# vt-asaplab/vPIN

Measured on AMD Instinct MI355X. Metric: R1CS constraints/sec, whole Spartan SNARK (sat proof + SPARK evaluation proof; vPIN point-mult + point-add instances), higher is better.
Workload: dtype u256 (integers mod q and mod p = 2^255-19, 32-bit limbs); 1 GPU; vPIN LeNet trace (layers L1..L7): 12 SNARKs per step; inputs=resident in HBM, parallelism=one trace per rank x 1 rank(s), no collective; 4 stream(s) per rank, table_slot_bytes=128

## Files before the change

### include/vpin_hip.h

```cpp
#ifndef VPIN_HIP_H
#define VPIN_HIP_H
#include <stddef.h>
#include <stdint.h>

#ifdef __cplusplus
extern "C" {
#endif

#define VPIN_OK 0
#define VPIN_EINVAL (-1)
#define VPIN_ENODEV (-2)
#define VPIN_ENOMEM (-3)
#define VPIN_EHIP (-4)
#define VPIN_ESHAPE (-5)
#define VPIN_EVERIFY (-6)

typedef struct vpin_ctx vpin_ctx;
typedef struct vpin_table vpin_table;

const char* vpin_strerror(int code);
const char* vpin_last_error(void);
int vpin_crash_line_set(const char* line, size_t n);
int vpin_abi_version(void);

// ... 39 lines not shown
int vpin_sc_quad_bind_round(vpin_ctx* ctx, vpin_table* A, vpin_table* B, const uint8_t r[32],
                            uint8_t out_e0_e2[64]);

int vpin_eq_table(vpin_ctx* ctx, const uint8_t* r, int ell, vpin_table** out);

int vpin_eq_suffix_tables(vpin_ctx* ctx, const uint8_t* tau, int ell, vpin_table** out);
int vpin_sc_cubic3_round(vpin_ctx* ctx, const vpin_table* pyramid, int ell, int level, vpin_table* Az,
                         vpin_table* Bz, vpin_table* Cz, uint8_t out_S0_S2_S3[96]);
int vpin_sc_cubic3_bind_round(vpin_ctx* ctx, const vpin_table* pyramid, int ell, int level, vpin_table* Az,
                              vpin_table* Bz, vpin_table* Cz, const uint8_t r[32], uint8_t out_S0_S2_S3[96]);
int vpin_sc_cubic3_lead_round(vpin_ctx* ctx, const vpin_table* pyramid, int ell, int level, vpin_table* Az,
                              vpin_table* Bz, vpin_table* Cz, const uint8_t* r, uint8_t out[96]);
int vpin_spark_batched_round(vpin_ctx* ctx, vpin_table* forest, size_t n, int ncirc, int level, size_t len,
                             const vpin_table* E, size_t e_off, const uint8_t* r, int lead, const vpin_table* derefs,
                             const vpin_table* vals, vpin_table* scratch, int first_fold, uint8_t* out);

typedef struct vpin_gens vpin_gens;
int vpin_gens_create(vpin_ctx* ctx, const uint8_t* gens_xyzt, size_t nb, vpin_gens** out);
int vpin_gens_map_stream(vpin_ctx* ctx, const uint8_t* stream64, size_t nb, uint8_t* out_xyzt);
int vpin_gens_shared(vpin_ctx* ctx, const char* label, const uint8_t* gens_xyzt, size_t nb, size_t budget_gb,
                     const vpin_gens** out);
void vpin_gens_shared_clear(void);
size_t vpin_gens_shared_bytes(int device);
void vpin_gens_free(vpin_ctx* ctx, vpin_gens* g);
size_t vpin_gens_count(const vpin_gens* g);
int vpin_gens_layout(const vpin_gens* g, size_t out[6]);
size_t vpin_gens_entry_bytes(void);
int vpin_hyrax_commit(vpin_ctx* ctx, const vpin_gens* g, const vpin_table* Z, const uint8_t* blinds,
                      size_t L, size_t blind_base, uint8_t* out_compressed );
int vpin_hyrax_commit_rows(vpin_ctx* ctx, const vpin_gens* g, const vpin_table* Z, size_t L, size_t row0, size_t nrows,
// ... 200 lines not shown
```

### vpin_amd/csrc/sc_dev.h

```cpp
#pragma once
#include <cstring>

#include "ctx.h"

namespace vpin {

#ifndef VPIN_SC_MIN_WAVES
#define VPIN_SC_MIN_WAVES 3
#endif
constexpr int kBlock = 256;
constexpr int kMinWaves = VPIN_SC_MIN_WAVES;
constexpr int kMaxBlocksCap = 16384;
inline int max_blocks() {
  static const int n = [] { const char* e = getenv("VPIN_SC_BLOCKS"); int v = e ? atoi(e) : 1024; return v < 1 ? 1 : v > kMaxBlocksCap ? kMaxBlocksCap : v; }();
  return n;
}


__device__ __forceinline__ fq comb_cubic(const fq& a, const fq& b, const fq& c, const fq& d) {
  return fq_mul(a, fq_sub(fq_mul(b, c), d));
}

template <int K>
struct Acc;
// ... 65 lines not shown
    fqw_mac(w[1], E, Y);
#ifndef VPIN_LAZY_NO_FLUSH
    if (++n == 7) flush(e);
#endif
#endif
  }
  __device__ __forceinline__ void flush(fq* e) {
    if (n == 0) return;
    e[0] = fq_add(e[0], fqw_reduce(w[0]));
    e[1] = fq_add(e[1], fqw_reduce(w[1]));
    fqw_zero(w[0]); fqw_zero(w[1]);
    n = 0;
  }
};

template <>
struct Acc<2> {
  static constexpr int NE = 2;
  fq e[2];
  __device__ __forceinline__ void init() { e[0] = e[1] = fq_zero(); }
  __device__ __forceinline__ void add_pair(fq* p, const fq* d) {
    e[0] = fq_add(e[0], fq_mul(p[0], p[1]));
#pragma unroll
    for (int k = 0; k < 2; k++) p[k] = fq_add(fq_add(p[k], d[k]), d[k]);
    e[1] = fq_add(e[1], fq_mul(p[0], p[1]));
  }
};

template <int K>
struct Tabs {
// ... 89 lines not shown
```

### vpin_amd/csrc/spark.cpp

```cpp
#include <cstdio>

#include "host/prover_common.h"
#include "gadget_dev.h"
#include "spark_dev.h"

namespace {

using namespace vpin_host;
using namespace vpin_prover;

static bool spark_trace() { static const bool on = getenv("VPIN_SPARK_TRACE") != nullptr; return on; }
struct TraceSpan {
  const char* name; Clock::time_point t0;
  explicit TraceSpan(const char* n) : name(n), t0(Clock::now()) {}
  ~TraceSpan() { if (spark_trace()) fprintf(stderr, "[spark] %-28s %8.3f ms\n", name, secs(t0, Clock::now()) * 1e3); }
};


struct SparkGens {
  std::vector<Point> g;
  std::map<size_t, std::unique_ptr<PcGens>> views;
};

static void spark_cache_free(vpin_ctx* c) {
// ... 216 lines not shown
  std::vector<Fq> dotp[3];
};

static void write_batched(Writer& w, const Batched& b) {
  w.u64(b.polys.size());
  for (size_t l = 0; l < b.polys.size(); l++) {
    w.u64(b.polys[l].size() / 3);
    for (size_t j = 0; j < b.polys[l].size() / 3; j++) w_scalars(w, &b.polys[l][3 * j], 3);
    w_scalars(w, b.claims_left[l].data(), b.claims_left[l].size());
    w_scalars(w, b.claims_right[l].data(), b.claims_right[l].size());
  }
  for (int k = 0; k < 3; k++) w_scalars(w, b.dotp[k].data(), b.dotp[k].size());
}

static inline size_t pyramid_offset(int ell, int k) { return ((size_t)1 << ell) - ((size_t)2 << (ell - k)); }

struct DotpCtx {
  const vpin_spark_decomm* d;
  const vpin::fq* comb_derefs;
  vpin::fq* scratch;
  Fq claims[6];
};

static int batched_prove(vpin_ctx* c, vpin::SparkForest& f, DotpCtx* dotp, Transcript& tr, Batched& out, std::vector<Fq>& rand,
                         const DistPlan* pl = nullptr, int npc_all = 0) {
  const int npc = pl ? npc_all : f.ncirc, ndotp = dotp ? 6 : 0;
  const bool is_mem = pl && npc_all == 4;
  const int nl = f.ncirc;
  const std::vector<int> no_halves;
  const std::vector<int>& my_halves = pl ? pl->dotp_of[pl->rank] : no_halves;
// ... 96 lines not shown
      for (auto& x : rho_inv) lead_ok = lead_ok && !x.is_zero();
      if (lead_ok) {
        std::vector<Fq> pre(k);
        Fq acc = one;
        for (int j = 0; j < k; j++) { pre[j] = acc; acc = acc * rho_inv[j]; }
        acc = acc.invert();
        for (int j = k - 1; j >= 0; j--) { Fq t = acc * rho_inv[j]; rho_inv[j] = acc * pre[j]; acc = t; }
      }
      Fq cn = Fq::zero();
      for (int t = 0; t < npc; t++) cn = cn + claims[t] * coeffs[t];
      const size_t tail_pairs = lead_ok ? vpin::spark_tail_pairs() : 0;
      if (pl && tail_pairs == 0) {
        vpin::set_last_error("one proof over several GPUs needs the persistent tail rounds", hipErrorUnknown);
        return VPIN_ESHAPE;
      }
      bool tail_on = false;
      int tail_j0 = 0;
      const int ninst = nl + ndl_here;
      if (fine) { auto t = Clock::now(); t_setup += secs(tl0, t); tl0 = t; }
      for (int j = 0; j < k; j++) {
        const size_t len = j == 0 ? h : (h >> (j - 1));
        const vpin::fq* E = runs ? pyr->d + pyramid_offset(k, j + 1) : nullptr;
        const uint8_t* rprev = j ? B(&r[j - 1]) : nullptr;
        if (!tail_on && (h >> (j + 1)) <= tail_pairs) {
          if (runs && (rc = vpin::spark_tail_launch(c, &f, layer_id, k, j, len, pyr->d, rprev, ndl_here ? dotp->d->N : 0,
                                                    ndl_here ? dotp->d->vals : nullptr,
                                                    ndl_here ? dotp->comb_derefs : nullptr, ndl_here ? dotp->scratch : nullptr,
                                                    halves, ndl_here)))
            return rc;
          tail_on = true;
          tail_j0 = j;
        }
        const Fq* res = nullptr;
        if (tail_on) {
          if (runs) {
            if ((rc = vpin::spark_tail_wait(c, j - tail_j0, ninst, nl))) return rc;
            res = reinterpret_cast<const Fq*>(vpin::spark_tail_sums(c));
          }
        } else if (runs) {
          if ((rc = vpin::spark_prod_round(c, &f, layer_id, len, E, rprev, ndl_here, lead_ok))) return rc;
          if (ndl_here && (rc = vpin::spark_dotp_round(c, dotp->d->N, dotp->d->vals, dotp->comb_derefs, dotp->scratch, len, j == 1, rprev, halves, ndl_here))) return rc;
          if ((rc = vpin::spark_wait_flag(c))) return rc;
          res = reinterpret_cast<const Fq*>(c->h_spark);
        }
        if (pl) {
          for (int t = 0; t < nl; t++) memcpy(&pack[3 * (size_t)t], res + 3 * (size_t)t, 96);
          for (int i = 0; i < ndl_here; i++) memcpy(&pack[3 * (size_t)(nl + i)], res + 3 * (size_t)((tail_on ? nl : 12) + i), 96);
          if ((rc = dist_exchange(c, *pl, is_mem, with_dotp, pack.data(), 3, res_all.data(),
                                  is_mem ? (tail_on ? "mem_tail_round" : "mem_round") : (tail_on ? "ops_tail_round" : "ops_round"))))
            return rc;
          res = res_all.data();
        }
        if (fine) { auto t = Clock::now(); (j == 0 ? t_first : t_rounds) += secs(tl0, t); if (k >= 11) fprintf(stderr, " w%.1f", secs(tl0, t) * 1e6); tl0 = t; }
        const Fq rho = rand[j], omr = one - rho;
        Fq S0 = Fq::zero(), S2 = Fq::zero(), S3 = Fq::zero(), T1 = Fq::zero(), Sinf = Fq::zero();
        if (lead_ok) {
          for (int t = 0; t < npc; t++) { S0 = S0 + res[3 * t] * coeffs[t]; Sinf = Sinf + res[3 * t + 1] * coeffs[t]; }
          T1 = (cn - omr * S0) * rho_inv[j];
// ... 810 lines not shown
  return 8 * 6 + 8 + 32 * ((size_t)1 << (s.v_ops / 2)) + 8 + 32 * ((size_t)1 << (s.v_mem / 2));
}

size_t vpin_snark_proof_max_bytes(const vpin_r1cs* inst) {
  if (!inst) return 0;
  Shape s = shape_of(inst->num_cons, inst->num_vars, inst->nnz);
  const size_t lgN = log2z(s.N), lgM = log2z(s.M);
  size_t b = vpin_sat_proof_max_bytes(inst->num_cons, inst->num_vars) + 96;
  b += 8 + 32 * ((size_t)1 << (s.v_derefs / 2)) + 64 * 32;
  b += lgN * (lgN * 104 + 64 + 24 * 32 + 64) + 18 * 32 + 64;
  b += lgM * (lgM * 104 + 64 + 8 * 32 + 64) + 64;
  b += 3 * (16 + 64 * 40 + 128 + 64) + 40 * 32 + 1024;
  return b;
}

int vpin_spark_prepare(vpin_ctx* c, size_t num_cons, size_t num_vars, size_t max_nnz) {
  if (!c || !vpin::is_pow2(num_cons) || !vpin::is_pow2(num_vars) || max_nnz == 0) return VPIN_EINVAL;
  (void)hipSetDevice(c->device);
  const size_t nnz[3] = {max_nnz, max_nnz, max_nnz};
  const Shape s = shape_of(num_cons, num_vars, nnz);
  const PcGens* g = nullptr;
  int rc = get_view(c, std::max(s.v_ops, s.v_mem), &g);
  if (!rc) {
    auto* sg = static_cast<SparkGens*>(c->spark_cache);
    std::vector<size_t> idx;
    for (size_t ell : {s.v_ops, s.v_mem, s.v_derefs}) {
      const size_t R = (size_t)1 << (ell - ell / 2);
      if (R + 1 < sg->g.size()) { idx.push_back(R); idx.push_back(R + 1); }
    }
#pragma omp parallel for schedule(dynamic, 1) num_threads(host_threads())
// ... 312 lines not shown
```

### vpin_amd/csrc/spark.hip

```cpp
#include <chrono>
#include <cstdlib>

#include "mailbox_dev.h"
#include "sc_dev.h"
#include "spark_dev.h"

namespace vpin {

__device__ __forceinline__ fq fq_r2() {
  fq r;
  r.v[0] = 0x449c0f01u; r.v[1] = 0xa40611e3u; r.v[2] = 0x68859347u; r.v[3] = 0xd00e1ba7u;
  r.v[4] = 0x17f5be65u; r.v[5] = 0xceec73d2u; r.v[6] = 0x7c309a3du; r.v[7] = 0x0399411bu;
  return r;
}
__device__ __forceinline__ fq fq_raw_u32(uint32_t x) {
  fq r = fq_zero();
  r.v[0] = x;
  return r;
}

__global__ __launch_bounds__(kBlock) void u32_to_fq_kernel(const uint32_t* __restrict__ src, fq* __restrict__ dst, size_t n) {
  const fq r2 = fq_r2();
  for (size_t i = (size_t)blockIdx.x * kBlock + threadIdx.x; i < n; i += (size_t)gridDim.x * kBlock) {
    uint32_t x = src[i];
// ... 7 lines not shown
  const int s = blockIdx.y;
  fq* dst = comb + (size_t)s * N;
  if (s >= 6) {
    for (size_t i = (size_t)blockIdx.x * kBlock + threadIdx.x; i < N; i += (size_t)gridDim.x * kBlock) fq_store(dst + i, fq_zero());
    return;
  }
  const uint32_t* a = idx + (size_t)(s < 3 ? s : 3 + s) * N;
  const fq* mem = s < 3 ? mem_rx : mem_ry;
  for (size_t i = (size_t)blockIdx.x * kBlock + threadIdx.x; i < N; i += (size_t)gridDim.x * kBlock)
    fq_store(dst + i, fq_load(mem + a[i]));
}

struct HashParams { fq r, r2, r2_boost, gamma; };
struct CircIds { int v[12]; };

__global__ __launch_bounds__(kBlock) void hash_ops_kernel(const uint32_t* __restrict__ idx, const fq* __restrict__ derefs, size_t N,
                                                          HashParams hp, fq* __restrict__ forest) {
  const int side = blockIdx.y / 3, m = blockIdx.y % 3;
  const uint32_t* addr = idx + (size_t)(side * 6 + m) * N;
  const uint32_t* ts = idx + (size_t)(side * 6 + 3 + m) * N;
  const fq* val = derefs + (size_t)(side * 3 + m) * N;
  fq* rd = forest + (size_t)(side * 6 + m) * 2 * N;
  fq* wr = forest + (size_t)(side * 6 + 3 + m) * 2 * N;
  const fq r2c = fq_r2();
  for (size_t i = (size_t)blockIdx.x * kBlock + threadIdx.x; i < N; i += (size_t)gridDim.x * kBlock) {
    fq h = fq_sub(fq_mul(fq_load(val + i), hp.r), hp.gamma);
    uint32_t a = addr[i], t = ts[i];
    if (a) h = fq_add(h, fq_mul(fq_raw_u32(a), r2c));
    if (t) h = fq_add(h, fq_mul(fq_raw_u32(t), hp.r2_boost));
    fq_store(rd + i, h);
    fq_store(wr + i, fq_add(h, hp.r2));
  }
}

__global__ __launch_bounds__(kBlock) void hash_mem_kernel(const uint32_t* __restrict__ audit_ts, const fq* __restrict__ mem_rx,
                                                          const fq* __restrict__ mem_ry, size_t M, HashParams hp,
                                                          fq* __restrict__ forest) {
  const int side = blockIdx.y;
  const fq* mem = side ? mem_ry : mem_rx;
  const uint32_t* ts = audit_ts + (size_t)side * M;
  fq* init = forest + (size_t)(2 * side) * 2 * M;
  fq* audit = forest + (size_t)(2 * side + 1) * 2 * M;
  const fq r2c = fq_r2();
  for (size_t i = (size_t)blockIdx.x * kBlock + threadIdx.x; i < M; i += (size_t)gridDim.x * kBlock) {
    fq h = fq_sub(fq_mul(fq_load(mem + i), hp.r), hp.gamma);
    if (i) h = fq_add(h, fq_mul(fq_raw_u32((uint32_t)i), r2c));
// ... 113 lines not shown
__global__ __launch_bounds__(kBlock) void take_strided_kernel(const fq* __restrict__ src, size_t nloc, size_t r0, size_t step,
                                                              fq* __restrict__ dst) {
  for (size_t k = (size_t)blockIdx.x * kBlock + threadIdx.x; k < nloc; k += (size_t)gridDim.x * kBlock)
    fq_store(dst + k, fq_load(src + r0 + k * step));
}

__global__ __launch_bounds__(kBlock) void tree_level_kernel(fq* __restrict__ forest, size_t stride, size_t src_off, size_t dst_off,
                                                            size_t h) {
  fq* t = forest + (size_t)blockIdx.y * stride;
  const fq* src = t + src_off;
  fq* dst = t + dst_off;
  for (size_t i = (size_t)blockIdx.x * kBlock + threadIdx.x; i < h; i += (size_t)gridDim.x * kBlock)
    fq_store(dst + i, fq_mul(fq_load(src + i), fq_load(src + h + i)));
}

__global__ __launch_bounds__(kBlock) void tree_level3_kernel(fq* __restrict__ forest, size_t stride, size_t src_off, size_t d1_off,
                                                             size_t d2_off, size_t d3_off, size_t h) {
  fq* t = forest + (size_t)blockIdx.y * stride;
  const fq* src = t + src_off;
  fq *d1 = t + d1_off, *d2 = t + d2_off, *d3 = t + d3_off;
  const size_t q = h / 4;
  for (size_t i = (size_t)blockIdx.x * kBlock + threadIdx.x; i < q; i += (size_t)gridDim.x * kBlock) {
    const fq a0 = fq_mul(fq_load(src + i), fq_load(src + h + i));
    const fq a1 = fq_mul(fq_load(src + q + i), fq_load(src + h + q + i));
    const fq a2 = fq_mul(fq_load(src + 2 * q + i), fq_load(src + h + 2 * q + i));
    const fq a3 = fq_mul(fq_load(src + 3 * q + i), fq_load(src + h + 3 * q + i));
    fq_store(d1 + i, a0); fq_store(d1 + q + i, a1); fq_store(d1 + 2 * q + i, a2); fq_store(d1 + 3 * q + i, a3);
    const fq b0 = fq_mul(a0, a2), b1 = fq_mul(a1, a3);
    fq_store(d2 + i, b0); fq_store(d2 + q + i, b1);
    fq_store(d3 + i, fq_mul(b0, b1));
  }
}

constexpr int kTopBlock = 1024;
__global__ __launch_bounds__(kTopBlock) void tree_top_kernel(fq* __restrict__ forest, size_t stride, size_t n2, size_t h0) {
  fq* t = forest + (size_t)blockIdx.x * stride;
  for (size_t h = h0; h >= 1; h >>= 1) {
    const fq* src = t + (n2 - 4 * h);
    fq* dst = t + (n2 - 2 * h);
    if (threadIdx.x < h) fq_store(dst + threadIdx.x, fq_mul(fq_load(src + threadIdx.x), fq_load(src + h + threadIdx.x)));
    __syncthreads();
  }
}


// ... 63 lines not shown
    }
  }
}


__device__ __forceinline__ void fold_pd2(const fq* src, fq* dst, size_t i, size_t q, const fq& r, fq& p, fq& d) {
  fq a0 = fq_load(src + i), a1 = fq_load(src + 2 * q + i);
  fq b0 = fq_load(src + q + i), b1 = fq_load(src + 3 * q + i);
  p = fq_add(a0, fq_mul(r, fq_sub(a1, a0)));
  fq hi = fq_add(b0, fq_mul(r, fq_sub(b1, b0)));
  fq_store(dst + i, p);
  fq_store(dst + q + i, hi);
  d = fq_sub(hi, p);
}

template <bool BIND, bool LEAD, bool BIG = false>
__global__ __launch_bounds__(kBlock, kMinWaves) void prod_round_kernel(fq* __restrict__ forest, size_t stride, size_t off, size_t h,
                                                                       const fq* __restrict__ E, size_t pairs, fq r, fq_const rc,
                                                                       Finisher fin) {
  __shared__ __attribute__((aligned(16))) uint32_t tt[8][8];
  if (BIND && LEAD) {
    if (threadIdx.x < 64) tt[threadIdx.x >> 3][threadIdx.x & 7] = rc.tt[threadIdx.x >> 3][threadIdx.x & 7];
    __syncthreads();
  }
  fq* A = forest + (size_t)blockIdx.y * stride + off;
  fq* B = A + h;
  Acc<4> acc;
  acc.init();
  LeadAcc lacc;
  if (LEAD) lacc.init();
  for (size_t i = (size_t)blockIdx.x * kBlock + threadIdx.x; i < pairs; i += (size_t)gridDim.x * kBlock) {
    fq u[3], p1, d1, p2, d2;
    if (BIND && LEAD) { fold_pd_c(A, i, pairs, tt, p1, d1); fold_pd_c(B, i, pairs, tt, p2, d2); }
    else if (BIND) { fold_pd(A, i, pairs, r, p1, d1); fold_pd(B, i, pairs, r, p2, d2); }
    else { load_pd(A, i, pairs, p1, d1); load_pd(B, i, pairs, p2, d2); }
    if (LEAD) {
      lacc.add(acc.e, fq_load(E + i), fq_mul(p1, p2), fq_mul(d1, d2));
    } else {
      acc.stage_bc(u, p1, d1, p2, d2);
      acc.stage_e(u, fq_load(E + i));
    }
  }
  if (LEAD) lacc.flush(acc.e);
  finish_block(acc.e, fin);
}

struct DotpPtrs { const fq* src[3]; fq* dst[3]; size_t src_stride[3]; };

template <bool BIND>
__global__ __launch_bounds__(kBlock, kMinWaves) void dotp_round_kernel(const fq* __restrict__ derefs, const fq* __restrict__ vals,
                                                                       size_t N, fq* __restrict__ scratch, bool from_scratch,
                                                                       size_t pairs, fq r, Finisher fin, CircIds kmap) {
  const int k = kmap.v[blockIdx.y], m = k >> 1, half = k & 1;
  const size_t hN = N / 2, q4 = N / 4;
  const fq* src[3];
  fq* dst[3];
#pragma unroll
  for (int t = 0; t < 3; t++) dst[t] = scratch + (size_t)(3 * blockIdx.y + t) * q4;
  if (from_scratch) {
// ... 291 lines not shown
  for (int m = 0; m < 3; m++) {
    const int k = h[2 * m + 1] > h[2 * m] ? 1 : 0;
    if (h[2 * m + k] >= d->N / 64) d->hot_col[m] = k ? v1 : v0;
  }
  return VPIN_OK;
}

int spark_gather_derefs(vpin_ctx* c, const vpin_spark_decomm* d, const fq* mem_rx, const fq* mem_ry, fq* comb) {
  ProfScope ps(c, VPIN_K_SPARK_BUILD, (double)d->N * (6 * 68.0 + 2 * 32.0));
  hipLaunchKernelGGL(gather_derefs_kernel, dim3(grid_for(d->N), 8), dim3(kBlock), 0, c->stream, (const uint32_t*)d->idx, d->N,
                     mem_rx, mem_ry, comb);
  VPIN_HIP_TRY(hipGetLastError());
  return VPIN_OK;
}

static int build_levels(vpin_ctx* c, SparkForest* f) {
  const size_t n2 = 2 * f->n;
  size_t h = f->n / 2;
  int l = 0;
  while (h > (size_t)kTopBlock) {
    if (h / 4 > (size_t)kTopBlock) {
      hipLaunchKernelGGL(tree_level3_kernel, dim3(grid_for(h / 4), f->ncirc), dim3(kBlock), 0, c->stream, f->base, f->stride(),
                         f->level_off(l), f->level_off(l + 1), f->level_off(l + 2), f->level_off(l + 3), h);
      h >>= 3;
      l += 3;
      continue;
    }
    hipLaunchKernelGGL(tree_level_kernel, dim3(grid_for(h), f->ncirc), dim3(kBlock), 0, c->stream, f->base, f->stride(),
                       f->level_off(l), f->level_off(l + 1), h);
    h >>= 1;
    l++;
  }
  if (h >= 1) hipLaunchKernelGGL(tree_top_kernel, dim3(f->ncirc), dim3(kTopBlock), 0, c->stream, f->base, f->stride(), n2, h);
  VPIN_HIP_TRY(hipGetLastError());
  return VPIN_OK;
}

int spark_build_forests(vpin_ctx* c, const vpin_spark_decomm* d, const fq* comb_derefs, const fq* mem_rx, const fq* mem_ry,
                        const uint8_t r_hash[32], const uint8_t r_hash_sqr[32], const uint8_t r_hash_sqr_boost[32],
                        const uint8_t gamma[32], SparkForest* ops, SparkForest* mem) {
  if (!c || !d || !ops || !mem || !ops->base || !mem->base) return VPIN_EINVAL;
  if (ops->n != d->N || mem->n != d->M || ops->ncirc != 12 || mem->ncirc != 4 || d->N < 2 || d->M < 2) return VPIN_ESHAPE;
  (void)hipSetDevice(c->device);
  HashParams hp;
  hp.r = load_host_fq(r_hash);
  hp.r2 = load_host_fq(r_hash_sqr);
  hp.r2_boost = load_host_fq(r_hash_sqr_boost);
  hp.gamma = load_host_fq(gamma);
  {
    ProfScope ps(c, VPIN_K_SPARK_BUILD, (double)d->N * (6 * (8.0 + 32.0) + 12 * 32.0 + 12 * 64.0) + (double)d->M * (2 * 36.0 + 4 * 32.0 + 4 * 64.0));
    hipLaunchKernelGGL(hash_ops_kernel, dim3(grid_for(d->N), 6), dim3(kBlock), 0, c->stream, (const uint32_t*)d->idx, comb_derefs,
                       d->N, hp, ops->base);
    hipLaunchKernelGGL(hash_mem_kernel, dim3(grid_for(d->M), 2), dim3(kBlock), 0, c->stream,
                       (const uint32_t*)(d->idx + 12 * d->N), mem_rx, mem_ry, d->M, hp, mem->base);
    VPIN_HIP_TRY(hipGetLastError());
    int rc = build_levels(c, ops);
    if (!rc) rc = build_levels(c, mem);
    if (rc) return rc;
  }
  return VPIN_OK;
}

__device__ __forceinline__ fq fq_wave_prod(fq a) {
#pragma unroll
  for (int off = 32; off >= 1; off >>= 1) a = fq_mul(a, fq_shfl_xor(a, off));
  return a;
}
__global__ __launch_bounds__(kBlock) void hash_mem_roots_kernel(const uint32_t* __restrict__ audit_ts, const fq* __restrict__ mem_rx,
                                                                const fq* __restrict__ mem_ry, size_t M, HashParams hp,
                                                                fq* __restrict__ parts) {
  const int side = blockIdx.y;
// ... 58 lines not shown
    ProfScope ps(c, VPIN_K_SPARK_BUILD, (double)d->M * 2 * 36.0);
    hipLaunchKernelGGL(hash_mem_roots_kernel, dim3((unsigned)np, 2), dim3(kBlock), 0, c->stream, (const uint32_t*)(d->idx + 12 * d->N), mem_rx,
                       mem_ry, d->M, hash_params(r_hash, r_hash_sqr, r_hash_sqr_boost, gamma), (fq*)parts.p);
  }
  hipLaunchKernelGGL(roots_finish_kernel, dim3(4), dim3(kBlock), 0, c->stream, (const fq*)parts.p, np, c->h_spark);
  VPIN_HIP_TRY(hipGetLastError());
  return spark_wait(c);
}

int spark_build_forest_ops(vpin_ctx* c, const vpin_spark_decomm* d, const fq* comb_derefs, const uint8_t r_hash[32],
                           const uint8_t r_hash_sqr[32], const uint8_t r_hash_sqr_boost[32], const uint8_t gamma[32], SparkForest* ops) {
  if (!c || !d || !ops || !ops->base || !comb_derefs) return VPIN_EINVAL;
  if (ops->n != d->N || ops->ncirc != 12 || d->N < 2) return VPIN_ESHAPE;
  (void)hipSetDevice(c->device);
  ProfScope ps(c, VPIN_K_SPARK_BUILD, (double)d->N * (6 * (8.0 + 32.0) + 12 * 32.0 + 12 * 64.0));
  hipLaunchKernelGGL(hash_ops_kernel, dim3(grid_for(d->N), 6), dim3(kBlock), 0, c->stream, (const uint32_t*)d->idx, comb_derefs, d->N,
                     hash_params(r_hash, r_hash_sqr, r_hash_sqr_boost, gamma), ops->base);
  VPIN_HIP_TRY(hipGetLastError());
  return build_levels(c, ops);
}
int spark_build_forest_mem(vpin_ctx* c, const vpin_spark_decomm* d, const fq* mem_rx, const fq* mem_ry, const uint8_t r_hash[32],
                           const uint8_t r_hash_sqr[32], const uint8_t r_hash_sqr_boost[32], const uint8_t gamma[32], SparkForest* mem) {
  if (!c || !d || !mem || !mem->base || !mem_rx || !mem_ry) return VPIN_EINVAL;
  if (mem->n != d->M || mem->ncirc != 4 || d->M < 2) return VPIN_ESHAPE;
  (void)hipSetDevice(c->device);
  ProfScope ps(c, VPIN_K_SPARK_BUILD, (double)d->M * (2 * 36.0 + 4 * 32.0 + 4 * 64.0));
  hipLaunchKernelGGL(hash_mem_kernel, dim3(grid_for(d->M), 2), dim3(kBlock), 0, c->stream, (const uint32_t*)(d->idx + 12 * d->N), mem_rx,
                     mem_ry, d->M, hash_params(r_hash, r_hash_sqr, r_hash_sqr_boost, gamma), mem->base);
  VPIN_HIP_TRY(hipGetLastError());
  return build_levels(c, mem);
}

int spark_build_forest_sub(vpin_ctx* c, const vpin_spark_decomm* d, const fq* comb_derefs, const fq* mem_rx, const fq* mem_ry,
                           const uint8_t r_hash[32], const uint8_t r_hash_sqr[32], const uint8_t r_hash_sqr_boost[32],
// ... 116 lines not shown
}

static inline size_t fused_finish_max() {
  static const size_t n = [] { const char* e = getenv("VPIN_SPARK_FUSED_FINISH_MAX"); long v = e ? atol(e) : 64; return (size_t)(v < 0 ? 0 : v); }();
  return n;
}

static int round_finish_launch(vpin_ctx* c, const fq* partials, int ncirc, int np, int ndotp, int nd) {
  hipLaunchKernelGGL(round_finish_kernel, dim3(1), dim3(kFinishBlock), 0, c->stream, partials, ncirc, np,
                     partials + (size_t)12 * kRoundBlocks * 3, ndotp, nd, c->h_spark, flag_ptr(c), c->spark_seq);
  VPIN_HIP_TRY(hipGetLastError());
  return VPIN_OK;
}

int spark_prod_round(vpin_ctx* c, const SparkForest* f, int level, size_t len, const fq* E, const uint8_t* r, int ndotp,
                     bool lead) {
  const bool with_dotp = ndotp > 0;
  if (!c || !f || !f->base || !E) return VPIN_EINVAL;
  const size_t h = f->n >> (level + 1);
  if (h == 0 || len > h || !is_pow2(len) || len < (r ? 4u : 2u) || f->ncirc > 12 || f->ncirc < 1 || ndotp < 0 || ndotp > 6) return VPIN_ESHAPE;
  int rc = spark_pinned(c);
  if (rc) return rc;
  (void)hipSetDevice(c->device);
  fq* partials = nullptr;
  if ((rc = round_partials(c, &partials))) return rc;
  const size_t pairs = r ? len / 4 : len / 2;
  const int grid = round_grid(pairs, f->ncirc, c->shared_device);
  const fq rr = r ? load_host_fq(r) : fq{};
  const fq_const rconst = (r && lead) ? make_fq_const(r) : fq_const{};
  c->spark_seq++;
  Finisher fin = make_finisher(c, partials, 0, f->ncirc + ndotp);
  const size_t group_blocks = (size_t)grid * f->ncirc + (with_dotp ? (size_t)round_grid(pairs, 6, c->shared_device) * ndotp : 0);
  fin.fused = group_blocks <= fused_finish_max() ? 1 : 0;
  c->round_split = fin.fused ? 0 : 1;
  c->round_split_grid = grid;
  c->round_split_ncirc = f->ncirc;
  c->round_group_ndotp = ndotp;
  {
    const double bytes = (double)f->ncirc * 2 * 32.0 * (r ? (double)len * 1.5 : (double)len) + 32.0 * (r ? (double)len * 1.5 : (double)len);
    ProfScope ps(c, VPIN_K_SPARK_ROUND, bytes, pairs >= ((size_t)1 << 20) ? VPIN_K_SPARK_ROUND_BIG : -1, (double)f->ncirc * (double)pairs);
#define VPIN_PROD_LAUNCH(B_, L_, G_)                                                                                              \
  hipLaunchKernelGGL((prod_round_kernel<B_, L_, G_>), dim3(grid, f->ncirc), dim3(kBlock), 0, c->stream, f->base, f->stride(), \
                     f->level_off(level), h, E, pairs, rr, rconst, fin)
    const bool big = lead && pairs >= ((size_t)1 << 20);
    if (r) { if (big) VPIN_PROD_LAUNCH(true, true, true); else if (lead) VPIN_PROD_LAUNCH(true, true, false); else VPIN_PROD_LAUNCH(true, false, false); }
    else { if (big) VPIN_PROD_LAUNCH(false, true, true); else if (lead) VPIN_PROD_LAUNCH(false, true, false); else VPIN_PROD_LAUNCH(false, false, false); }
#undef VPIN_PROD_LAUNCH
  }
  VPIN_HIP_TRY(hipGetLastError());
  if (!fin.fused && !with_dotp) return round_finish_launch(c, partials, f->ncirc, grid, 0, 0);
  return VPIN_OK;
}

int spark_dotp_round(vpin_ctx* c, size_t N, const fq* vals, const fq* comb_derefs, fq* scratch, size_t len, bool first_fold,
                     const uint8_t* r, const int* halves, int ndotp) {
  if (!c || !vals || !comb_derefs || !scratch || ndotp < 1 || ndotp > 6) return VPIN_EINVAL;
  if (ndotp != c->round_group_ndotp) return VPIN_ESHAPE;
  CircIds kmap{};
  for (int i = 0; i < ndotp; i++) {
    kmap.v[i] = halves ? halves[i] : i;
    if (kmap.v[i] < 0 || kmap.v[i] > 5) return VPIN_EINVAL;
  }
  if (len > N / 2 || !is_pow2(len) || len < (r ? 4u : 2u) || (first_fold && (!r || len != N / 2))) return VPIN_ESHAPE;
  int rc = spark_pinned(c);
  if (rc) return rc;
// ... 434 lines not shown
  const bool with_dotp = derefs != nullptr;
  if (with_dotp && (!vals || !scratch || ncirc != 12 || level != 0)) return VPIN_EINVAL;
  if (forest->len < (size_t)ncirc * 2 * n) return VPIN_ESHAPE;
  const size_t pairs = r ? len / 4 : len / 2;
  if (e_off + pairs > E->len) return VPIN_ESHAPE;
  if (with_dotp && (derefs->len < 6 * n || vals->len < 3 * n || scratch->len < 18 * (n / 4))) return VPIN_ESHAPE;
  SparkForest f;
  f.base = forest->d; f.n = n; f.ncirc = ncirc;
  int rc = spark_prod_round(c, &f, level, len, E->d + e_off, r, with_dotp ? 6 : 0, lead != 0);
  if (!rc && with_dotp) rc = spark_dotp_round(c, n, vals->d, derefs->d, scratch->d, len, first_fold != 0, r);
  if (!rc) rc = spark_wait_flag(c);
  if (rc) return rc;
  memcpy(out, c->h_spark, (size_t)(ncirc + (with_dotp ? 6 : 0)) * 96);
  return VPIN_OK;
}
```

### vpin_amd/csrc/spark_dev.h

```cpp
#pragma once
#include <mutex>

#include "ctx.h"

struct vpin_spark_decomm {
  size_t num_cons = 0, num_vars = 0, num_inputs = 0;
  size_t nx = 0, ny = 0, N = 0, M = 0;
  uint32_t* idx = nullptr;
  vpin::fq* vals = nullptr;
  vpin_table* comb_ops = nullptr;
  vpin_table* comb_mem = nullptr;
  std::mutex comb_mu;
  bool comb_unpooled = false;
  uint32_t hot_col[3] = {0xffffffffu, 0xffffffffu, 0xffffffffu};
};

namespace vpin {

constexpr size_t kSparkPinned = 8192;
constexpr int kSparkMaxInst = 18;
constexpr size_t kSparkHostTop = 32;

int spark_pinned(vpin_ctx* c);

int spark_trace_timestamps(vpin_ctx* c, const uint32_t* addr, size_t n, size_t M, uint32_t* ts, uint32_t* audit);
int spark_check_bounds(vpin_ctx* c, const uint32_t* a, size_t nnz, uint32_t limit, uint32_t* d_bad);

int spark_u32_to_fq(vpin_ctx* c, const uint32_t* src, fq* dst, size_t n);
int spark_comb_tables(vpin_ctx* c, vpin_spark_decomm* d);
int spark_comb_make(vpin_ctx* c, const vpin_spark_decomm* d, vpin_table** ops, vpin_table** mem, bool pooled = true);
void spark_comb_release(vpin_ctx* c, vpin_spark_decomm* d, bool to_driver = false);

int spark_gather_derefs(vpin_ctx* c, const vpin_spark_decomm* d, const fq* mem_rx, const fq* mem_ry, fq* comb);
int spark_find_hot_cols(vpin_ctx* c, vpin_spark_decomm* d);

struct SparkForest {
  fq* base = nullptr;
  size_t n = 0;
  int ncirc = 0;
  size_t stride() const { return 2 * n; }
  size_t level_off(int l) const { return 2 * n - ((2 * n) >> l); }
};

int spark_build_forests(vpin_ctx* c, const vpin_spark_decomm* d, const fq* comb_derefs, const fq* mem_rx, const fq* mem_ry,
                        const uint8_t r_hash[32], const uint8_t r_hash_sqr[32], const uint8_t r_hash_sqr_boost[32],
                        const uint8_t gamma[32], SparkForest* ops, SparkForest* mem);

int spark_build_forest_ops(vpin_ctx* c, const vpin_spark_decomm* d, const fq* comb_derefs, const uint8_t r_hash[32],
                           const uint8_t r_hash_sqr[32], const uint8_t r_hash_sqr_boost[32], const uint8_t gamma[32], SparkForest* ops);
int spark_mem_roots(vpin_ctx* c, const vpin_spark_decomm* d, const fq* mem_rx, const fq* mem_ry, const uint8_t r_hash[32],
                    const uint8_t r_hash_sqr[32], const uint8_t r_hash_sqr_boost[32], const uint8_t gamma[32]);
int spark_build_forest_mem(vpin_ctx* c, const vpin_spark_decomm* d, const fq* mem_rx, const fq* mem_ry, const uint8_t r_hash[32],
                           const uint8_t r_hash_sqr[32], const uint8_t r_hash_sqr_boost[32], const uint8_t gamma[32], SparkForest* mem);

int spark_build_forest_sub(vpin_ctx* c, const vpin_spark_decomm* d, const fq* comb_derefs, const fq* mem_rx, const fq* mem_ry,
                           const uint8_t r_hash[32], const uint8_t r_hash_sqr[32], const uint8_t r_hash_sqr_boost[32],
                           const uint8_t gamma[32], SparkForest* f, const int* ids, bool is_mem);

int spark_fetch_tops(vpin_ctx* c, const SparkForest* f, size_t cnt);

int spark_prod_round(vpin_ctx* c, const SparkForest* f, int level, size_t len, const fq* E, const uint8_t* r, int ndotp,
                     bool lead = false);

int spark_dotp_round(vpin_ctx* c, size_t N, const fq* vals, const fq* comb_derefs, fq* scratch, size_t len, bool first_fold,
                     const uint8_t* r, const int* halves = nullptr, int ndotp = 6);

int spark_wait_flag(vpin_ctx* c);

int spark_collect(vpin_ctx* c, const SparkForest* f, int level, const vpin_spark_decomm* d, const fq* comb_derefs,
                  const fq* scratch, bool with_dotp, bool folded);

int spark_triple_sums(vpin_ctx* c, const vpin_spark_decomm* d, const fq* comb_derefs, const int* halves = nullptr, int nh = 6);
int spark_triple_sums_raw(vpin_ctx* c, const fq* comb_derefs, const fq* vals, size_t N, const int* halves = nullptr, int nh = 6);

size_t spark_tail_pairs();
int spark_tail_launch(vpin_ctx* c, const SparkForest* f, int level, int k, int j0, size_t len0, const fq* pyr, const uint8_t* r_prev,
                      size_t N, const fq* vals, const fq* comb_derefs, fq* scratch, const int* halves = nullptr, int ndotp = 6);
// ... 20 lines not shown
```

Baseline: 73.67 million constraints/s.

## Derive SPARK write-set leaf tables from read-set tables instead of materializing them

The ops forest's write-set leaves are the read-set hash plus r2. They are no longer stored at hash time, and the first three tree levels for write circuits are built from the read leaves plus r2 in registers. In the leaf-layer sumcheck rounds only the 6 read circuits are processed. An extra accumulator (p1+p2) lets the host derive the write circuits' round evaluations algebraically. Write tables are materialized lazily only for the small tail rounds, cutting leaf-level memory traffic roughly in half at the cost of extra host math and complexity.

```diff
diff --git a/include/vpin_hip.h b/include/vpin_hip.h
--- a/include/vpin_hip.h
+++ b/include/vpin_hip.h
@@ -77,6 +77,10 @@
 int vpin_spark_batched_round(vpin_ctx* ctx, vpin_table* forest, size_t n, int ncirc, int level, size_t len,
                              const vpin_table* E, size_t e_off, const uint8_t* r, int lead, const vpin_table* derefs,
                              const vpin_table* vals, vpin_table* scratch, int first_fold, uint8_t* out);
+int vpin_spark_leaf_round(vpin_ctx* ctx, vpin_table* forest, size_t n, size_t len, const vpin_table* E, size_t e_off,
+                          const uint8_t* r, uint8_t* out);
+int vpin_spark_leaf_derive(const uint8_t rd[96], const uint8_t r2[32], const uint8_t sum_e[32], uint8_t out[64]);
+int vpin_spark_leaf_write_tables(vpin_ctx* ctx, vpin_table* forest, size_t n, size_t len, const uint8_t r2[32]);
 
 typedef struct vpin_gens vpin_gens;
 int vpin_gens_create(vpin_ctx* ctx, const uint8_t* gens_xyzt, size_t nb, vpin_gens** out);
diff --git a/vpin_amd/csrc/sc_dev.h b/vpin_amd/csrc/sc_dev.h
--- a/vpin_amd/csrc/sc_dev.h
+++ b/vpin_amd/csrc/sc_dev.h
@@ -103,6 +103,27 @@
   }
 };
 
+struct LeadAcc3 {
+  fq_wide w[3];
+  int n;
+  __device__ __forceinline__ void init() { fqw_zero(w[0]); fqw_zero(w[1]); fqw_zero(w[2]); n = 0; }
+  __device__ __forceinline__ void add(fq* e, const fq& E, const fq& X, const fq& Y, const fq& Z) {
+    fqw_mac(w[0], E, X);
+    fqw_mac(w[1], E, Y);
+    fqw_mac(w[2], E, Z);
+    if (++n == 7) flush(e);
+  }
+  __device__ __forceinline__ void flush(fq* e) {
+    if (n == 0) return;
+#pragma unroll
+    for (int k = 0; k < 3; k++) {
+      e[k] = fq_add(e[k], fqw_reduce(w[k]));
+      fqw_zero(w[k]);
+    }
+    n = 0;
+  }
+};
+
 template <>
 struct Acc<2> {
   static constexpr int NE = 2;
diff --git a/vpin_amd/csrc/spark.cpp b/vpin_amd/csrc/spark.cpp
--- a/vpin_amd/csrc/spark.cpp
+++ b/vpin_amd/csrc/spark.cpp
@@ -254,6 +254,25 @@
 }
 
 static inline size_t pyramid_offset(int ell, int k) { return ((size_t)1 << ell) - ((size_t)2 << (ell - k)); }
+
+static inline void leaf_derive(const Fq rd[3], const Fq& r2, const Fq& sum_e, Fq wr[2]) {
+  wr[0] = rd[0] + r2 * (rd[2] + r2 * sum_e);
+  wr[1] = rd[1];
+}
+static inline Fq eq_suffix_sum(const Fq* rho, int j, int k) {
+  Fq s = Fq::one();
+  for (int i = j + 1; i < k; i++) s = s * ((Fq::one() - rho[i]) + rho[i]);
+  return s;
+}
+static void leaf_expand(const Fq* rd6, const Fq& r2, const Fq& sum_e, Fq* out12) {
+  for (int y = 0; y < 6; y++) {
+    const int rdc = y + 3 * (y / 3);
+    Fq wr[2];
+    leaf_derive(rd6 + 3 * y, r2, sum_e, wr);
+    out12[3 * rdc] = rd6[3 * y]; out12[3 * rdc + 1] = rd6[3 * y + 1]; out12[3 * rdc + 2] = Fq::zero();
+    out12[3 * (rdc + 3)] = wr[0]; out12[3 * (rdc + 3) + 1] = wr[1]; out12[3 * (rdc + 3) + 2] = Fq::zero();
+  }
+}
 
 struct DotpCtx {
   const vpin_spark_decomm* d;
@@ -380,6 +399,11 @@
         vpin::set_last_error("one proof over several GPUs needs the persistent tail rounds", hipErrorUnknown);
         return VPIN_ESHAPE;
       }
+      const bool wr_derived = !pl && f.wr_derived && layer_id == 0;
+      const bool derive = wr_derived && lead_ok && tail_pairs > 0;
+      Fq leaf_r2 = Fq::zero();
+      if (wr_derived) memcpy(&leaf_r2, &f.r2, 32);
+      if (wr_derived && !derive && (rc = vpin::spark_leaf_write_tables(c, &f, h))) return rc;
       bool tail_on = false;
       int tail_j0 = 0;
       const int ninst = nl + ndl_here;
@@ -389,6 +413,7 @@
         const vpin::fq* E = runs ? pyr->d + pyramid_offset(k, j + 1) : nullptr;
         const uint8_t* rprev = j ? B(&r[j - 1]) : nullptr;
         if (!tail_on && (h >> (j + 1)) <= tail_pairs) {
+          if (derive && (rc = vpin::spark_leaf_write_tables(c, &f, len))) return rc;
           if (runs && (rc = vpin::spark_tail_launch(c, &f, layer_id, k, j, len, pyr->d, rprev, ndl_here ? dotp->d->N : 0,
                                                     ndl_here ? dotp->d->vals : nullptr,
                                                     ndl_here ? dotp->comb_derefs : nullptr, ndl_here ? dotp->scratch : nullptr,
@@ -404,10 +429,15 @@
             res = reinterpret_cast<const Fq*>(vpin::spark_tail_sums(c));
           }
         } else if (runs) {
-          if ((rc = vpin::spark_prod_round(c, &f, layer_id, len, E, rprev, ndl_here, lead_ok))) return rc;
+          if ((rc = vpin::spark_prod_round(c, &f, layer_id, len, E, rprev, ndl_here, lead_ok, derive))) return rc;
           if (ndl_here && (rc = vpin::spark_dotp_round(c, dotp->d->N, dotp->d->vals, dotp->comb_derefs, dotp->scratch, len, j == 1, rprev, halves, ndl_here))) return rc;
           if ((rc = vpin::spark_wait_flag(c))) return rc;
           res = reinterpret_cast<const Fq*>(c->h_spark);
+          if (derive) {
+            leaf_expand(res, leaf_r2, eq_suffix_sum(rand.data(), j, k), res_all.data());
+            for (int i = 0; i < 3 * ndl_here; i++) res_all[3 * 12 + i] = res[3 * 12 + i];
+            res = res_all.data();
+          }
         }
         if (pl) {
           for (int t = 0; t < nl; t++) memcpy(&pack[3 * (size_t)t], res + 3 * (size_t)t, 96);
@@ -1248,6 +1278,15 @@
   return b;
 }
 
+int vpin_spark_leaf_derive(const uint8_t rd[96], const uint8_t r2[32], const uint8_t sum_e[32], uint8_t out[64]) {
+  if (!rd || !r2 || !sum_e || !out) return VPIN_EINVAL;
+  Fq a[3], b, s, w[2];
+  memcpy(a, rd, 96); memcpy(&b, r2, 32); memcpy(&s, sum_e, 32);
+  leaf_derive(a, b, s, w);
+  memcpy(out, w, 64);
+  return VPIN_OK;
+}
+
 int vpin_spark_prepare(vpin_ctx* c, size_t num_cons, size_t num_vars, size_t max_nnz) {
   if (!c || !vpin::is_pow2(num_cons) || !vpin::is_pow2(num_vars) || max_nnz == 0) return VPIN_EINVAL;
   (void)hipSetDevice(c->device);
diff --git a/vpin_amd/csrc/spark.hip b/vpin_amd/csrc/spark.hip
--- a/vpin_amd/csrc/spark.hip
+++ b/vpin_amd/csrc/spark.hip
@@ -45,6 +45,7 @@
 struct HashParams { fq r, r2, r2_boost, gamma; };
 struct CircIds { int v[12]; };
 
+template <bool WR>
 __global__ __launch_bounds__(kBlock) void hash_ops_kernel(const uint32_t* __restrict__ idx, const fq* __restrict__ derefs, size_t N,
                                                           HashParams hp, fq* __restrict__ forest) {
   const int side = blockIdx.y / 3, m = blockIdx.y % 3;
@@ -60,7 +61,7 @@
     if (a) h = fq_add(h, fq_mul(fq_raw_u32(a), r2c));
     if (t) h = fq_add(h, fq_mul(fq_raw_u32(t), hp.r2_boost));
     fq_store(rd + i, h);
-    fq_store(wr + i, fq_add(h, hp.r2));
+    if (WR) fq_store(wr + i, fq_add(h, hp.r2));
   }
 }
 
@@ -204,21 +205,44 @@
     fq_store(dst + i, fq_mul(fq_load(src + i), fq_load(src + h + i)));
 }
 
+__device__ __forceinline__ void tree3_store(const fq* x, fq* __restrict__ d1, fq* __restrict__ d2, fq* __restrict__ d3, size_t i, size_t q) {
+  const fq a0 = fq_mul(x[0], x[4]);
+  const fq a1 = fq_mul(x[1], x[5]);
+  const fq a2 = fq_mul(x[2], x[6]);
+  const fq a3 = fq_mul(x[3], x[7]);
+  fq_store(d1 + i, a0); fq_store(d1 + q + i, a1); fq_store(d1 + 2 * q + i, a2); fq_store(d1 + 3 * q + i, a3);
+  const fq b0 = fq_mul(a0, a2), b1 = fq_mul(a1, a3);
+  fq_store(d2 + i, b0); fq_store(d2 + q + i, b1);
+  fq_store(d3 + i, fq_mul(b0, b1));
+}
 __global__ __launch_bounds__(kBlock) void tree_level3_kernel(fq* __restrict__ forest, size_t stride, size_t src_off, size_t d1_off,
                                                              size_t d2_off, size_t d3_off, size_t h) {
   fq* t = forest + (size_t)blockIdx.y * stride;
   const fq* src = t + src_off;
-  fq *d1 = t + d1_off, *d2 = t + d2_off, *d3 = t + d3_off;
   const size_t q = h / 4;
   for (size_t i = (size_t)blockIdx.x * kBlock + threadIdx.x; i < q; i += (size_t)gridDim.x * kBlock) {
-    const fq a0 = fq_mul(fq_load(src + i), fq_load(src + h + i));
-    const fq a1 = fq_mul(fq_load(src + q + i), fq_load(src + h + q + i));
-    const fq a2 = fq_mul(fq_load(src + 2 * q + i), fq_load(src + h + 2 * q + i));
-    const fq a3 = fq_mul(fq_load(src + 3 * q + i), fq_load(src + h + 3 * q + i));
-    fq_store(d1 + i, a0); fq_store(d1 + q + i, a1); fq_store(d1 + 2 * q + i, a2); fq_store(d1 + 3 * q + i, a3);
-    const fq b0 = fq_mul(a0, a2), b1 = fq_mul(a1, a3);
-    fq_store(d2 + i, b0); fq_store(d2 + q + i, b1);
-    fq_store(d3 + i, fq_mul(b0, b1));
+    fq x[8];
+#pragma unroll
+    for (int j = 0; j < 8; j++) x[j] = fq_load(src + j * q + i);
+    tree3_store(x, t + d1_off, t + d2_off, t + d3_off, i, q);
+  }
+}
+
+__global__ __launch_bounds__(kBlock) void tree_level3_rw_kernel(fq* __restrict__ forest, size_t stride, size_t d1_off, size_t d2_off,
+                                                                size_t d3_off, size_t h, fq r2) {
+  const bool wr = (blockIdx.y % 6) >= 3;
+  fq* t = forest + (size_t)blockIdx.y * stride;
+  const fq* src = wr ? t - 3 * stride : t;
+  const size_t q = h / 4;
+  for (size_t i = (size_t)blockIdx.x * kBlock + threadIdx.x; i < q; i += (size_t)gridDim.x * kBlock) {
+    fq x[8];
+#pragma unroll
+    for (int j = 0; j < 8; j++) x[j] = fq_load(src + j * q + i);
+    if (wr) {
+#pragma unroll
+      for (int j = 0; j < 8; j++) x[j] = fq_add(x[j], r2);
+    }
+    tree3_store(x, t + d1_off, t + d2_off, t + d3_off, i, q);
   }
 }
 
@@ -312,35 +336,51 @@
   d = fq_sub(hi, p);
 }
 
-template <bool BIND, bool LEAD, bool BIG = false>
+template <bool BIND, bool LEAD, bool BIG = false, bool LEAF = false>
 __global__ __launch_bounds__(kBlock, kMinWaves) void prod_round_kernel(fq* __restrict__ forest, size_t stride, size_t off, size_t h,
                                                                        const fq* __restrict__ E, size_t pairs, fq r, fq_const rc,
                                                                        Finisher fin) {
+  static_assert(!LEAF || LEAD, "the leaf-layer form exists for the leading-coefficient rounds only");
   __shared__ __attribute__((aligned(16))) uint32_t tt[8][8];
   if (BIND && LEAD) {
     if (threadIdx.x < 64) tt[threadIdx.x >> 3][threadIdx.x & 7] = rc.tt[threadIdx.x >> 3][threadIdx.x & 7];
     __syncthreads();
   }
-  fq* A = forest + (size_t)blockIdx.y * stride + off;
+  const size_t circ = LEAF ? (size_t)blockIdx.y + 3 * (blockIdx.y / 3) : (size_t)blockIdx.y;
+  fq* A = forest + circ * stride + off;
   fq* B = A + h;
   Acc<4> acc;
   acc.init();
   LeadAcc lacc;
-  if (LEAD) lacc.init();
+  LeadAcc3 lacc3;
+  if (LEAF) lacc3.init();
+  else if (LEAD) lacc.init();
   for (size_t i = (size_t)blockIdx.x * kBlock + threadIdx.x; i < pairs; i += (size_t)gridDim.x * kBlock) {
     fq u[3], p1, d1, p2, d2;
     if (BIND && LEAD) { fold_pd_c(A, i, pairs, tt, p1, d1); fold_pd_c(B, i, pairs, tt, p2, d2); }
     else if (BIND) { fold_pd(A, i, pairs, r, p1, d1); fold_pd(B, i, pairs, r, p2, d2); }
     else { load_pd(A, i, pairs, p1, d1); load_pd(B, i, pairs, p2, d2); }
-    if (LEAD) {
+    if (LEAF) {
+      lacc3.add(acc.e, fq_load(E + i), fq_mul(p1, p2), fq_mul(d1, d2), fq_add(p1, p2));
+    } else if (LEAD) {
       lacc.add(acc.e, fq_load(E + i), fq_mul(p1, p2), fq_mul(d1, d2));
     } else {
       acc.stage_bc(u, p1, d1, p2, d2);
       acc.stage_e(u, fq_load(E + i));
     }
   }
-  if (LEAD) lacc.flush(acc.e);
+  if (LEAF) lacc3.flush(acc.e);
+  else if (LEAD) lacc.flush(acc.e);
   finish_block(acc.e, fin);
+}
+
+__global__ __launch_bounds__(kBlock) void leaf_write_tables_kernel(fq* __restrict__ forest, size_t stride, size_t h, size_t len, fq r2) {
+  const fq* rd = forest + ((size_t)blockIdx.y + 3 * (blockIdx.y / 3)) * stride;
+  fq* wr = forest + ((size_t)blockIdx.y + 3 * (blockIdx.y / 3) + 3) * stride;
+  for (size_t i = (size_t)blockIdx.x * kBlock + threadIdx.x; i < 2 * len; i += (size_t)gridDim.x * kBlock) {
+    const size_t j = i < len ? i : h + (i - len);
+    fq_store(wr + j, fq_add(fq_load(rd + j), r2));
+  }
 }
 
 struct DotpPtrs { const fq* src[3]; fq* dst[3]; size_t src_stride[3]; };
@@ -662,10 +702,19 @@
   return VPIN_OK;
 }
 
-static int build_levels(vpin_ctx* c, SparkForest* f) {
+static inline bool first_pass_is_level3(size_t n) { return n / 8 > (size_t)kTopBlock; }
+
+static int build_levels(vpin_ctx* c, SparkForest* f, const fq* r2 = nullptr) {
   const size_t n2 = 2 * f->n;
   size_t h = f->n / 2;
   int l = 0;
+  if (r2) {
+    if (f->ncirc != 12 || !first_pass_is_level3(f->n)) return VPIN_ESHAPE;
+    hipLaunchKernelGGL(tree_level3_rw_kernel, dim3(grid_for(h / 4), 12), dim3(kBlock), 0, c->stream, f->base, f->stride(),
+                       f->level_off(1), f->level_off(2), f->level_off(3), h, *r2);
+    h >>= 3;
+    l = 3;
+  }
   while (h > (size_t)kTopBlock) {
     if (h / 4 > (size_t)kTopBlock) {
       hipLaunchKernelGGL(tree_level3_kernel, dim3(grid_for(h / 4), f->ncirc), dim3(kBlock), 0, c->stream, f->base, f->stride(),
@@ -682,6 +731,20 @@
   if (h >= 1) hipLaunchKernelGGL(tree_top_kernel, dim3(f->ncirc), dim3(kTopBlock), 0, c->stream, f->base, f->stride(), n2, h);
   VPIN_HIP_TRY(hipGetLastError());
   return VPIN_OK;
+}
+
+static int build_ops_levels(vpin_ctx* c, const vpin_spark_decomm* d, const fq* comb_derefs, const HashParams& hp, SparkForest* ops) {
+  const bool in_regs = first_pass_is_level3(d->N);
+  if (in_regs)
+    hipLaunchKernelGGL((hash_ops_kernel<false>), dim3(grid_for(d->N), 6), dim3(kBlock), 0, c->stream, (const uint32_t*)d->idx, comb_derefs,
+                       d->N, hp, ops->base);
+  else
+    hipLaunchKernelGGL((hash_ops_kernel<true>), dim3(grid_for(d->N), 6), dim3(kBlock), 0, c->stream, (const uint32_t*)d->idx, comb_derefs,
+                       d->N, hp, ops->base);
+  VPIN_HIP_TRY(hipGetLastError());
+  ops->wr_derived = true;
+  ops->r2 = hp.r2;
+  return build_levels(c, ops, in_regs ? &hp.r2 : nullptr);
 }
 
 int spark_build_forests(vpin_ctx* c, const vpin_spark_decomm* d, const fq* comb_derefs, const fq* mem_rx, const fq* mem_ry,
@@ -697,12 +760,10 @@
   hp.gamma = load_host_fq(gamma);
   {
     ProfScope ps(c, VPIN_K_SPARK_BUILD, (double)d->N * (6 * (8.0 + 32.0) + 12 * 32.0 + 12 * 64.0) + (double)d->M * (2 * 36.0 + 4 * 32.0 + 4 * 64.0));
-    hipLaunchKernelGGL(hash_ops_kernel, dim3(grid_for(d->N), 6), dim3(kBlock), 0, c->stream, (const uint32_t*)d->idx, comb_derefs,
-                       d->N, hp, ops->base);
     hipLaunchKernelGGL(hash_mem_kernel, dim3(grid_for(d->M), 2), dim3(kBlock), 0, c->stream,
                        (const uint32_t*)(d->idx + 12 * d->N), mem_rx, mem_ry, d->M, hp, mem->base);
     VPIN_HIP_TRY(hipGetLastError());
-    int rc = build_levels(c, ops);
+    int rc = build_ops_levels(c, d, comb_derefs, hp, ops);
     if (!rc) rc = build_levels(c, mem);
     if (rc) return rc;
   }
@@ -791,10 +852,7 @@
   if (ops->n != d->N || ops->ncirc != 12 || d->N < 2) return VPIN_ESHAPE;
   (void)hipSetDevice(c->device);
   ProfScope ps(c, VPIN_K_SPARK_BUILD, (double)d->N * (6 * (8.0 + 32.0) + 12 * 32.0 + 12 * 64.0));
-  hipLaunchKernelGGL(hash_ops_kernel, dim3(grid_for(d->N), 6), dim3(kBlock), 0, c->stream, (const uint32_t*)d->idx, comb_derefs, d->N,
-                     hash_params(r_hash, r_hash_sqr, r_hash_sqr_boost, gamma), ops->base);
-  VPIN_HIP_TRY(hipGetLastError());
-  return build_levels(c, ops);
+  return build_ops_levels(c, d, comb_derefs, hash_params(r_hash, r_hash_sqr, r_hash_sqr_boost, gamma), ops);
 }
 int spark_build_forest_mem(vpin_ctx* c, const vpin_spark_decomm* d, const fq* mem_rx, const fq* mem_ry, const uint8_t r_hash[32],
                            const uint8_t r_hash_sqr[32], const uint8_t r_hash_sqr_boost[32], const uint8_t gamma[32], SparkForest* mem) {
@@ -941,9 +999,11 @@
 }
 
 int spark_prod_round(vpin_ctx* c, const SparkForest* f, int level, size_t len, const fq* E, const uint8_t* r, int ndotp,
-                     bool lead) {
+                     bool lead, bool leaf) {
   const bool with_dotp = ndotp > 0;
   if (!c || !f || !f->base || !E) return VPIN_EINVAL;
+  if (leaf && (!lead || level != 0 || f->ncirc != 12)) return VPIN_EINVAL;
+  const int ncirc = leaf ? 6 : f->ncirc;
   const size_t h = f->n >> (level + 1);
   if (h == 0 || len > h || !is_pow2(len) || len < (r ? 4u : 2u) || f->ncirc > 12 || f->ncirc < 1 || ndotp < 0 || ndotp > 6) return VPIN_ESHAPE;
   int rc = spark_pinned(c);
@@ -952,30 +1012,44 @@
   fq* partials = nullptr;
   if ((rc = round_partials(c, &partials))) return rc;
   const size_t pairs = r ? len / 4 : len / 2;
-  const int grid = round_grid(pairs, f->ncirc, c->shared_device);
+  const int grid = round_grid(pairs, ncirc, c->shared_device);
   const fq rr = r ? load_host_fq(r) : fq{};
   const fq_const rconst = (r && lead) ? make_fq_const(r) : fq_const{};
   c->spark_seq++;
-  Finisher fin = make_finisher(c, partials, 0, f->ncirc + ndotp);
-  const size_t group_blocks = (size_t)grid * f->ncirc + (with_dotp ? (size_t)round_grid(pairs, 6, c->shared_device) * ndotp : 0);
+  Finisher fin = make_finisher(c, partials, 0, ncirc + ndotp);
+  const size_t group_blocks = (size_t)grid * ncirc + (with_dotp ? (size_t)round_grid(pairs, 6, c->shared_device) * ndotp : 0);
   fin.fused = group_blocks <= fused_finish_max() ? 1 : 0;
   c->round_split = fin.fused ? 0 : 1;
   c->round_split_grid = grid;
-  c->round_split_ncirc = f->ncirc;
+  c->round_split_ncirc = ncirc;
   c->round_group_ndotp = ndotp;
   {
-    const double bytes = (double)f->ncirc * 2 * 32.0 * (r ? (double)len * 1.5 : (double)len) + 32.0 * (r ? (double)len * 1.5 : (double)len);
-    ProfScope ps(c, VPIN_K_SPARK_ROUND, bytes, pairs >= ((size_t)1 << 20) ? VPIN_K_SPARK_ROUND_BIG : -1, (double)f->ncirc * (double)pairs);
-#define VPIN_PROD_LAUNCH(B_, L_, G_)                                                                                              \
-  hipLaunchKernelGGL((prod_round_kernel<B_, L_, G_>), dim3(grid, f->ncirc), dim3(kBlock), 0, c->stream, f->base, f->stride(), \
+    const double bytes = (double)ncirc * 2 * 32.0 * (r ? (double)len * 1.5 : (double)len) + 32.0 * (r ? (double)len * 1.5 : (double)len);
+    ProfScope ps(c, VPIN_K_SPARK_ROUND, bytes, pairs >= ((size_t)1 << 20) ? VPIN_K_SPARK_ROUND_BIG : -1, (double)ncirc * (double)pairs);
+#define VPIN_PROD_LAUNCH(B_, L_, G_, F_)                                                                                      \
+  hipLaunchKernelGGL((prod_round_kernel<B_, L_, G_, F_>), dim3(grid, ncirc), dim3(kBlock), 0, c->stream, f->base, f->stride(), \
                      f->level_off(level), h, E, pairs, rr, rconst, fin)
     const bool big = lead && pairs >= ((size_t)1 << 20);
-    if (r) { if (big) VPIN_PROD_LAUNCH(true, true, true); else if (lead) VPIN_PROD_LAUNCH(true, true, false); else VPIN_PROD_LAUNCH(true, false, false); }
-    else { if (big) VPIN_PROD_LAUNCH(false, true, true); else if (lead) VPIN_PROD_LAUNCH(false, true, false); else VPIN_PROD_LAUNCH(false, false, false); }
+    if (leaf) {
+      if (r) { if (big) VPIN_PROD_LAUNCH(true, true, true, true); else VPIN_PROD_LAUNCH(true, true, false, true); }
+      else { if (big) VPIN_PROD_LAUNCH(false, true, true, true); else VPIN_PROD_LAUNCH(false, true, false, true); }
+    } else if (r) { if (big) VPIN_PROD_LAUNCH(true, true, true, false); else if (lead) VPIN_PROD_LAUNCH(true, true, false, false); else VPIN_PROD_LAUNCH(true, false, false, false); }
+    else { if (big) VPIN_PROD_LAUNCH(false, true, true, false); else if (lead) VPIN_PROD_LAUNCH(false, true, false, false); else VPIN_PROD_LAUNCH(false, false, false, false); }
 #undef VPIN_PROD_LAUNCH
   }
   VPIN_HIP_TRY(hipGetLastError());
-  if (!fin.fused && !with_dotp) return round_finish_launch(c, partials, f->ncirc, grid, 0, 0);
+  if (!fin.fused && !with_dotp) return round_finish_launch(c, partials, ncirc, grid, 0, 0);
+  return VPIN_OK;
+}
+
+int spark_leaf_write_tables(vpin_ctx* c, const SparkForest* f, size_t len) {
+  if (!c || !f || !f->base || f->ncirc != 12 || !f->wr_derived) return VPIN_EINVAL;
+  const size_t h = f->n / 2;
+  if (len < 1 || len > h) return VPIN_ESHAPE;
+  (void)hipSetDevice(c->device);
+  ProfScope ps(c, VPIN_K_SPARK_ROUND, 6 * 2 * 64.0 * (double)len);
+  hipLaunchKernelGGL(leaf_write_tables_kernel, dim3(grid_for(2 * len), 6), dim3(kBlock), 0, c->stream, f->base, f->stride(), h, len, f->r2);
+  VPIN_HIP_TRY(hipGetLastError());
   return VPIN_OK;
 }
 
@@ -1440,3 +1514,30 @@
   memcpy(out, c->h_spark, (size_t)(ncirc + (with_dotp ? 6 : 0)) * 96);
   return VPIN_OK;
 }
+
+
+extern "C" int vpin_spark_leaf_round(vpin_ctx* c, vpin_table* forest, size_t n, size_t len, const vpin_table* E, size_t e_off,
+                                     const uint8_t* r, uint8_t* out) {
+  using namespace vpin;
+  if (!c || !forest || !E || !out || !is_pow2(n) || n < 4) return VPIN_EINVAL;
+  if (forest->len < (size_t)12 * 2 * n) return VPIN_ESHAPE;
+  const size_t pairs = r ? len / 4 : len / 2;
+  if (e_off + pairs > E->len) return VPIN_ESHAPE;
+  SparkForest f;
+  f.base = forest->d; f.n = n; f.ncirc = 12;
+  int rc = spark_prod_round(c, &f, 0, len, E->d + e_off, r, 0, true, true);
+  if (!rc) rc = spark_wait_flag(c);
+  if (rc) return rc;
+  memcpy(out, c->h_spark, (size_t)6 * 96);
+  return VPIN_OK;
+}
+
+extern "C" int vpin_spark_leaf_write_tables(vpin_ctx* c, vpin_table* forest, size_t n, size_t len, const uint8_t r2[32]) {
+  using namespace vpin;
+  if (!c || !forest || !r2 || !is_pow2(n) || n < 4) return VPIN_EINVAL;
+  if (forest->len < (size_t)12 * 2 * n) return VPIN_ESHAPE;
+  SparkForest f;
+  f.base = forest->d; f.n = n; f.ncirc = 12; f.wr_derived = true; f.r2 = load_host_fq(r2);
+  int rc = spark_leaf_write_tables(c, &f, len);
+  return rc ? rc : spark_wait(c);
+}
diff --git a/vpin_amd/csrc/spark_dev.h b/vpin_amd/csrc/spark_dev.h
--- a/vpin_amd/csrc/spark_dev.h
+++ b/vpin_amd/csrc/spark_dev.h
@@ -38,6 +38,8 @@
   fq* base = nullptr;
   size_t n = 0;
   int ncirc = 0;
+  bool wr_derived = false;
+  fq r2{};
   size_t stride() const { return 2 * n; }
   size_t level_off(int l) const { return 2 * n - ((2 * n) >> l); }
 };
@@ -60,7 +62,8 @@
 int spark_fetch_tops(vpin_ctx* c, const SparkForest* f, size_t cnt);
 
 int spark_prod_round(vpin_ctx* c, const SparkForest* f, int level, size_t len, const fq* E, const uint8_t* r, int ndotp,
-                     bool lead = false);
+                     bool lead = false, bool leaf = false);
+int spark_leaf_write_tables(vpin_ctx* c, const SparkForest* f, size_t len);
 
 int spark_dotp_round(vpin_ctx* c, size_t N, const fq* vals, const fq* comb_derefs, fq* scratch, size_t len, bool first_fold,
                      const uint8_t* r, const int* halves = nullptr, int ndotp = 6);
```

New measurement: 73.44 million constraints/s. Within noise of the previous version (-0.3%).
